# andygrove/datafusion-archive

Hardware: NVIDIA H100
Metric: rows/s filter+agg over 1e8-row Arrow batch (C2: SELECT a FROM t WHERE a>0.5, Float64) (higher is better)
Workload: dtype f64

## Files before the change

datafusion_archive_b200/csrc/api.cu:

```cuda
#include <dlfcn.h>
#include <nccl.h>
#include <sched.h>
#include <sys/syscall.h>
#include <unistd.h>

#include <algorithm>
#include <memory>

#include "common.cuh"

namespace dfgpu {

static thread_local std::string g_last_error;
void set_last_error(const std::string& m) { g_last_error = m; }

const char* dtype_name(int dt) {
  switch (dt) {
    case DFGPU_BOOL: return "Boolean";
    case DFGPU_INT8: return "Int8";
    case DFGPU_INT16: return "Int16";
    case DFGPU_INT32: return "Int32";
    case DFGPU_INT64: return "Int64";
    case DFGPU_UINT8: return "UInt8";
    case DFGPU_UINT16: return "UInt16";
// ... 104 lines not shown
  if (!prof_on) return -1;
  const int s = prof_next;
  prof_next = (prof_next + 1) % kProfRing;
  if (!prof_ev[s][0]) {
    DF_CUDA(cudaEventCreate(&prof_ev[s][0]));
    DF_CUDA(cudaEventCreate(&prof_ev[s][1]));
  }
  if (prof_pending[s]) {
    float ms = 0;
    DF_CUDA(cudaEventSynchronize(prof_ev[s][1]));
    DF_CUDA(cudaEventElapsedTime(&ms, prof_ev[s][0], prof_ev[s][1]));
    prof_ms += ms;
    prof_n++;
    prof_pending[s] = false;
  }
  DF_CUDA(cudaEventRecord(prof_ev[s][0], stream));
  return s;
}
void dfgpu_ctx::prof_end(int s) {
  if (s < 0) return;
  DF_CUDA(cudaEventRecord(prof_ev[s][1], stream));
  prof_pending[s] = true;
}
void dfgpu_ctx::prof_drain() {
  for (int s = 0; s < kProfRing; s++) {
    if (!prof_pending[s]) continue;
    float ms = 0;
    DF_CUDA(cudaEventSynchronize(prof_ev[s][1]));
    DF_CUDA(cudaEventElapsedTime(&ms, prof_ev[s][0], prof_ev[s][1]));
    prof_ms += ms;
    prof_n++;
    prof_pending[s] = false;
  }
}

extern "C" int dfgpu_profile_enable(dfgpu_ctx* ctx, int on) {
  return guarded([&] {
    ctx->use();
    ctx->prof_drain();
    ctx->prof_on = on != 0;
    ctx->prof_ms = 0.0;
    ctx->prof_n = 0;
  });
}
extern "C" int dfgpu_profile_get(dfgpu_ctx* ctx, double* kernel_ms, int64_t* launches) {
  return guarded([&] {
    ctx->use();
    ctx->prof_drain();
    *kernel_ms = ctx->prof_ms;
    *launches = ctx->prof_n;
  });
}

dfgpu_batch::~dfgpu_batch() {
  if (!ctx || !owns) return;
  cudaSetDevice(ctx->device);
  for (auto& c : cols) {
    ctx->free(c.values);
    ctx->free(c.validity);
    ctx->free(c.offsets);
  }
}
void* dfgpu_ctx::host_alloc(size_t bytes) {
  if (bytes == 0) bytes = 8;
  HostBlock* best = nullptr;
  for (auto& b : host_blocks)
    if (!b.used && b.bytes >= bytes && b.bytes <= 2 * bytes + (1 << 20) && (!best || b.bytes < best->bytes)) best = &b;
  if (best) {
    best->used = true;
    return best->p;
  }
  void* p = nullptr;
  DF_CUDA(cudaMallocHost(&p, bytes));
  host_blocks.push_back(HostBlock{p, bytes, true});
  return p;
}
void dfgpu_ctx::host_release(void* p) {
  for (auto& b : host_blocks)
    if (b.p == p) b.used = false;
}

dfgpu_result::~dfgpu_result() {
  if (!ctx) return;
  cudaSetDevice(ctx->device);
  if (on_host) {
    for (auto& c : cols) ctx->host_release(c.values);
    return;
  }
  for (auto& c : cols) {
    ctx->free(c.values);
    ctx->free(c.validity);
    ctx->free(c.offsets);
  }
}

extern "C" int dfgpu_abi_version(void) { return DFGPU_ABI_VERSION; }
extern "C" const char* dfgpu_last_error(void) { return g_last_error.c_str(); }

extern "C" int dfgpu_device_count(int* out) {
  return guarded([&] {
    int n = 0;
    cudaError_t e = cudaGetDeviceCount(&n);
    if (e != cudaSuccess) {
      cudaGetLastError();
      n = 0;
    }
    *out = n;
  });
}

static void bind_to_gpu_numa_node(int device) {
  if (const char* e = getenv("DFGPU_NUMA")) if (atoi(e) == 0) return;
  char bus[64] = {0};
  if (cudaDeviceGetPCIBusId(bus, sizeof(bus), device) != cudaSuccess) { cudaGetLastError(); return; }
  for (char* c = bus; *c; c++) *c = char(tolower((unsigned char)*c));
  int node = -1;
  {
    FILE* f = fopen((std::string("/sys/bus/pci/devices/") + bus + "/numa_node").c_str(), "r");
    if (!f) return;
    if (fscanf(f, "%d", &node) != 1) node = -1;
    fclose(f);
  }
  if (node < 0) {
    if (getenv("DFGPU_TRACE")) fprintf(stderr, "[dfgpu trace] device %d (%s): sysfs reports no NUMA node\n", device, bus);
    return;
  }
  FILE* f = fopen(("/sys/devices/system/node/node" + std::to_string(node) + "/cpulist").c_str(), "r");
  if (!f) return;
  char list[4096] = {0};
  const bool got = fgets(list, sizeof(list), f) != nullptr;
  fclose(f);
  if (!got) return;
  cpu_set_t set;
  CPU_ZERO(&set);
  int ncpu = 0;
  for (char* tok = strtok(list, ",\n"); tok; tok = strtok(nullptr, ",\n")) {
    int a = 0, b = 0;
// ... 7 lines not shown
  if (getenv("DFGPU_TRACE")) fprintf(stderr, "[dfgpu trace] device %d (%s) -> NUMA node %d, %d cpus, sched_setaffinity rc=%d\n", device, bus, node, ncpu, rc_aff);
  unsigned long mask[16] = {0};
  if (node < int(sizeof(mask) * 8)) {
    mask[node / (8 * sizeof(unsigned long))] |= 1ul << (node % (8 * sizeof(unsigned long)));
    syscall(SYS_set_mempolicy, 1 , mask, sizeof(mask) * 8);
  }
}

extern "C" int dfgpu_init(int device, dfgpu_ctx** out) {
  return guarded([&] {
    if (!out) fail(DFGPU_ERR_GENERAL, "dfgpu_init: null out");
    int n = 0;
    cudaError_t e = cudaGetDeviceCount(&n);
    if (e != cudaSuccess || n == 0) {
      cudaGetLastError();
      fail(DFGPU_ERR_CUDA, "no CUDA device available: this engine has no CPU fallback");
    }
    if (device < 0 || device >= n) fail(DFGPU_ERR_CUDA, "device ordinal " + std::to_string(device) + " out of range");
    auto ctx = std::make_unique<dfgpu_ctx>();
    ctx->device = device;
    ctx->use();
    bind_to_gpu_numa_node(device);
    cudaDeviceProp prop;
    DF_CUDA(cudaGetDeviceProperties(&prop, device));
    if (prop.major != 9 || prop.minor != 0)
      fail(DFGPU_ERR_CUDA, std::string("device '") + prop.name + "' is sm_" + std::to_string(prop.major * 10 + prop.minor) +
                               "; this library is built for sm_90a (H100) only");
    ctx->sm_count = prop.multiProcessorCount;
    ctx->device_mem_bytes = prop.totalGlobalMem;
    if (const char* e = getenv("DFGPU_FP_KERNEL")) ctx->force_direct_kernel = std::string(e) == "direct";
    DF_CUDA(cudaStreamCreateWithFlags(&ctx->stream, cudaStreamNonBlocking));
    DF_CUDA(cudaStreamCreateWithFlags(&ctx->stream_in, cudaStreamNonBlocking));
    DF_CUDA(cudaStreamCreateWithFlags(&ctx->stream_out, cudaStreamNonBlocking));
    DF_CUDA(cudaEventCreate(&ctx->ev_start));
    DF_CUDA(cudaEventCreate(&ctx->ev_stop));
    cudaMemPool_t pool;
    DF_CUDA(cudaDeviceGetDefaultMemPool(&pool, device));
    uint64_t thresh = ~0ull;
    DF_CUDA(cudaMemPoolSetAttribute(pool, cudaMemPoolAttrReleaseThreshold, &thresh));
    DF_CUDA(cudaMalloc(&ctx->d_scratch, 64 * 8));
    DF_CUDA(cudaMemset(ctx->d_scratch, 0, 64 * 8));
    DF_CUDA(cudaMallocHost(&ctx->h_scratch, 64 * 8));
    *out = ctx.release();
  });
}

extern "C" int dfgpu_comm_destroy(dfgpu_ctx* ctx);

extern "C" int dfgpu_shutdown(dfgpu_ctx* ctx) {
  return guarded([&] {
    if (!ctx) return;
    ctx->use();
    cudaStreamSynchronize(ctx->stream);
    dfgpu_comm_destroy(ctx);
    ctx->release_cached();
    if (ctx->flush_buf) cudaFree(ctx->flush_buf);
    for (int i = 0; i < 2; i++) {
      if (ctx->stage[i]) cudaFreeHost(ctx->stage[i]);
      if (ctx->stage_ev[i]) cudaEventDestroy(ctx->stage_ev[i]);
    }
    for (int i = 0; i < dfgpu_ctx::kProfRing; i++)
      for (int j = 0; j < 2; j++)
        if (ctx->prof_ev[i][j]) cudaEventDestroy(ctx->prof_ev[i][j]);
    for (auto& b : ctx->host_blocks) cudaFreeHost(b.p);
    cudaStreamDestroy(ctx->stream_in);
    cudaStreamDestroy(ctx->stream_out);
    cudaFree(ctx->d_scratch);
    cudaFreeHost(ctx->h_scratch);
    cudaEventDestroy(ctx->ev_start);
    cudaEventDestroy(ctx->ev_stop);
    cudaStreamDestroy(ctx->stream);
    delete ctx;
  });
}

extern "C" int dfgpu_sync(dfgpu_ctx* ctx) {
  return guarded([&] {
    ctx->use();
    DF_CUDA(cudaStreamSynchronize(ctx->stream));
  });
}

extern "C" int dfgpu_host_alloc(size_t bytes, void** out) {
  return guarded([&] { DF_CUDA(cudaMallocHost(out, bytes ? bytes : 8)); });
}
extern "C" int dfgpu_host_free(void* p) {
  return guarded([&] {
    if (p) DF_CUDA(cudaFreeHost(p));
  });
}

extern "C" int dfgpu_timer_start(dfgpu_ctx* ctx) {
  return guarded([&] {
    ctx->use();
    DF_CUDA(cudaEventRecord(ctx->ev_start, ctx->stream));
  });
}
extern "C" int dfgpu_timer_stop(dfgpu_ctx* ctx, float* ms) {
  return guarded([&] {
    ctx->use();
    DF_CUDA(cudaEventRecord(ctx->ev_stop, ctx->stream));
    DF_CUDA(cudaEventSynchronize(ctx->ev_stop));
    DF_CUDA(cudaEventElapsedTime(ms, ctx->ev_start, ctx->ev_stop));
  });
}

// ... 85 lines not shown
        for (uint8_t byte : tmp) valid += __builtin_popcount(byte);
        d.null_count = c.len - valid;
        if (d.null_count > 0) {
          d.validity = (uint8_t*)ctx->alloc(tmp.size());
          h2d(ctx, d.validity, tmp.data(), tmp.size());
          DF_CUDA(cudaStreamSynchronize(ctx->stream));
        }
      }
      const int w = dtype_width(c.dtype);
      if (w > 0) {
        d.values_bytes = size_t(c.len) * size_t(w);
        d.values = ctx->alloc(d.values_bytes);
        if (c.len > 0) {
          if (!c.values) fail(DFGPU_ERR_GENERAL, "null values buffer");
          h2d(ctx, d.values, static_cast<const uint8_t*>(c.values) + size_t(c.offset) * size_t(w), d.values_bytes);
        }
      } else if (c.dtype == DFGPU_BOOL) {
        std::vector<uint8_t> bits = c.len > 0 ? rebase_bits(static_cast<const uint8_t*>(c.values), c.offset, c.len) : std::vector<uint8_t>();
        d.values_bytes = bits.size();
        d.values = ctx->alloc(d.values_bytes);
        if (!bits.empty()) {
          h2d(ctx, d.values, bits.data(), bits.size());
          DF_CUDA(cudaStreamSynchronize(ctx->stream));
        }
      } else if (c.dtype == DFGPU_UTF8) {
        if (!c.offsets) fail(DFGPU_ERR_GENERAL, "Utf8 column without offsets buffer");
        d.offsets = (int32_t*)ctx->alloc(size_t(c.len + 1) * 4);
        h2d(ctx, d.offsets, c.offsets + c.offset, size_t(c.len + 1) * 4);
        const int32_t lo = c.offsets[c.offset], hi = c.offsets[c.offset + c.len];
        if (hi < lo || hi > c.values_bytes) fail(DFGPU_ERR_GENERAL, "corrupt Utf8 offsets");
        d.values_bytes = size_t(hi - lo);
        d.values = ctx->alloc((d.values_bytes + 15) & ~size_t(15));
        if (hi > lo) h2d(ctx, d.values, static_cast<const uint8_t*>(c.values) + lo, size_t(hi - lo));
        rebase_offsets(ctx, d.offsets, c.len + 1, lo);
      } else {
        fail(DFGPU_ERR_NOT_IMPLEMENTED, std::string("unsupported column type ") + std::to_string(c.dtype));
      }
      b->cols.push_back(d);
    }
    DF_CUDA(cudaStreamSynchronize(ctx->stream));
    *out = b.release();
  });
}

extern "C" int dfgpu_batch_rows(const dfgpu_batch* b, int64_t* nrows) {
  *nrows = b->nrows;
  return 0;
}
extern "C" int dfgpu_batch_free(dfgpu_batch* b) {
  return guarded([&] { delete b; });
}

extern "C" int dfgpu_result_shape(const dfgpu_result* r, int64_t* nrows, int* ncols) {
  *nrows = r->nrows;
  *ncols = int(r->cols.size());
  return 0;
}
extern "C" int dfgpu_result_col_dtype(const dfgpu_result* r, int i, int32_t* dtype) {
  return guarded([&] {
    if (i < 0 || size_t(i) >= r->cols.size()) fail(DFGPU_ERR_INVALID_COLUMN, "result column out of range");
    *dtype = r->cols[size_t(i)].dtype;
  });
}
extern "C" int dfgpu_result_col_bytes(const dfgpu_result* r, int i, int64_t* nbytes) {
  return guarded([&] {
    if (i < 0 || size_t(i) >= r->cols.size()) fail(DFGPU_ERR_INVALID_COLUMN, "result column out of range");
    const DevColumn& c = r->cols[size_t(i)];
    const int w = dtype_width(c.dtype);
    *nbytes = w ? r->nrows * w : int64_t(c.values_bytes);
  });
}
extern "C" int dfgpu_result_col_nulls(const dfgpu_result* r, int i, int64_t* nulls) {
  return guarded([&] {
    if (i < 0 || size_t(i) >= r->cols.size()) fail(DFGPU_ERR_INVALID_COLUMN, "result column out of range");
    *nulls = r->cols[size_t(i)].null_count;
  });
}
extern "C" int dfgpu_result_copy_col(const dfgpu_result* r, int i, void* dst_values, uint8_t* dst_validity, int32_t* dst_offsets) {
  return guarded([&] {
    if (i < 0 || size_t(i) >= r->cols.size()) fail(DFGPU_ERR_INVALID_COLUMN, "result column out of range");
    dfgpu_ctx* ctx = r->ctx;
    ctx->use();
    const DevColumn& c = r->cols[size_t(i)];
    const int w = dtype_width(c.dtype);
    const size_t nb = w ? size_t(r->nrows) * size_t(w) : c.values_bytes;
    if (r->on_host) {
      if (nb && dst_values) memcpy(dst_values, c.values, nb);
      if (dst_validity) memset(dst_validity, 0xff, size_t(r->nrows + 7) / 8);
      return;
    }
    if (nb && dst_values) DF_CUDA(cudaMemcpyAsync(dst_values, c.values, nb, cudaMemcpyDeviceToHost, ctx->stream));
    if (dst_validity) {
      const size_t vb = size_t(r->nrows + 7) / 8;
      if (c.validity) DF_CUDA(cudaMemcpyAsync(dst_validity, c.validity, vb, cudaMemcpyDeviceToHost, ctx->stream));
      else memset(dst_validity, 0xff, vb);
    }
    if (dst_offsets && c.offsets)
      DF_CUDA(cudaMemcpyAsync(dst_offsets, c.offsets, size_t(r->nrows + 1) * 4, cudaMemcpyDeviceToHost, ctx->stream));
    DF_CUDA(cudaStreamSynchronize(ctx->stream));
  });
}
extern "C" int dfgpu_result_col_device_ptr(const dfgpu_result* r, int i, const void** dptr) {
  return guarded([&] {
    if (i < 0 || size_t(i) >= r->cols.size()) fail(DFGPU_ERR_INVALID_COLUMN, "result column out of range");
    if (r->on_host) fail(DFGPU_ERR_GENERAL, "result lives in host memory: use dfgpu_result_col_host_ptr");
    *dptr = r->cols[size_t(i)].values;
  });
}
extern "C" int dfgpu_result_on_host(const dfgpu_result* r, int* on_host) {
  return guarded([&] {
    if (!r || !on_host) fail(DFGPU_ERR_GENERAL, "dfgpu_result_on_host: null argument");
    *on_host = r->on_host ? 1 : 0;
  });
}
extern "C" int dfgpu_result_col_host_ptr(const dfgpu_result* r, int i, const void** hptr) {
  return guarded([&] {
    if (i < 0 || size_t(i) >= r->cols.size()) fail(DFGPU_ERR_INVALID_COLUMN, "result column out of range");
    if (!r->on_host) fail(DFGPU_ERR_GENERAL, "result lives in device memory: use dfgpu_result_copy_col");
    *hptr = r->cols[size_t(i)].values;
  });
}
extern "C" int dfgpu_result_free(dfgpu_result* r) {
  return guarded([&] { delete r; });
}

namespace {

struct NcclApi {
  void* h = nullptr;
  ncclResult_t (*GetUniqueId)(ncclUniqueId*) = nullptr;
  ncclResult_t (*CommInitRank)(ncclComm_t*, int, ncclUniqueId, int) = nullptr;
  ncclResult_t (*CommDestroy)(ncclComm_t) = nullptr;
  ncclResult_t (*AllGather)(const void*, void*, size_t, ncclDataType_t, ncclComm_t, cudaStream_t) = nullptr;
  ncclResult_t (*AllReduce)(const void*, void*, size_t, ncclDataType_t, ncclRedOp_t, ncclComm_t, cudaStream_t) = nullptr;
  ncclResult_t (*Send)(const void*, size_t, ncclDataType_t, int, ncclComm_t, cudaStream_t) = nullptr;
  ncclResult_t (*Recv)(void*, size_t, ncclDataType_t, int, ncclComm_t, cudaStream_t) = nullptr;
  ncclResult_t (*Broadcast)(const void*, void*, size_t, ncclDataType_t, int, ncclComm_t, cudaStream_t) = nullptr;
  ncclResult_t (*GroupStart)() = nullptr;
  ncclResult_t (*GroupEnd)() = nullptr;
  const char* (*GetErrorString)(ncclResult_t) = nullptr;
};

NcclApi& nccl() {
  static NcclApi api;
  if (api.h) return api;
  void* h = dlopen("libnccl.so.2", RTLD_NOW | RTLD_NOLOAD);
  if (!h) h = dlopen("libnccl.so.2", RTLD_NOW);
  if (!h) h = dlopen("libnccl.so", RTLD_NOW);
  if (!h) fail(DFGPU_ERR_CUDA, std::string("cannot load libnccl: ") + dlerror());
#define LOAD(N)                                                     \
  *(void**)(&api.N) = dlsym(h, "nccl" #N);                          \
  if (!api.N) fail(DFGPU_ERR_CUDA, "libnccl is missing symbol nccl" #N);
  LOAD(GetUniqueId) LOAD(CommInitRank) LOAD(CommDestroy) LOAD(AllGather) LOAD(AllReduce) LOAD(GroupStart) LOAD(GroupEnd)
  LOAD(Send) LOAD(Recv) LOAD(Broadcast)
  LOAD(GetErrorString)
#undef LOAD
  api.h = h;
  return api;
}

#define DF_NCCL(expr)                                                                                        \
  do {                                                                                                       \
    ncclResult_t _r = (expr);                                                                                \
    if (_r != ncclSuccess) fail(DFGPU_ERR_CUDA, std::string("NCCL error: ") + nccl().GetErrorString(_r) + " (" #expr ")"); \
  } while (0)

}

extern "C" int dfgpu_comm_unique_id(uint8_t out_id[128]) {
  return guarded([&] {
    static_assert(sizeof(ncclUniqueId) == 128, "ncclUniqueId size");
// ... 115 lines not shown
```

datafusion_archive_b200/csrc/common.cuh:

```cuda
#pragma once
#include <cuda_runtime.h>

#include <cstdint>
#include <cstdio>
#include <cstring>
#include <string>
#include <map>
#include <unordered_map>
#include <vector>

#include "../../include/dfgpu.h"

namespace dfgpu {

struct Error {
  int code;
  std::string msg;
};
[[noreturn]] inline void fail(int code, const std::string& m) { throw Error{code, m}; }

void set_last_error(const std::string& m);

#define DF_CUDA(expr)                                                                              \
  do {                                                                                             \
// ... 13 lines not shown
    set_last_error(e.msg);
    return e.code;
  } catch (const std::exception& e) {
    set_last_error(std::string("internal: ") + e.what());
    return DFGPU_ERR_INTERNAL;
  }
}

const char* dtype_name(int dt);
int dtype_width(int dt);
inline bool is_signed_int(int dt) { return dt >= DFGPU_INT8 && dt <= DFGPU_INT64; }
inline bool is_unsigned_int(int dt) { return dt >= DFGPU_UINT8 && dt <= DFGPU_UINT64; }
inline bool is_int(int dt) { return dt >= DFGPU_INT8 && dt <= DFGPU_UINT64; }
inline bool is_float(int dt) { return dt == DFGPU_FLOAT32 || dt == DFGPU_FLOAT64; }
inline bool is_numeric(int dt) { return dt >= DFGPU_INT8 && dt <= DFGPU_FLOAT64; }
inline bool is_numeric8(int dt) { return dt == DFGPU_FLOAT64 || dt == DFGPU_INT64 || dt == DFGPU_UINT64; }
inline bool is_numeric4or8(int dt) { return is_numeric8(dt) || dt == DFGPU_FLOAT32 || dt == DFGPU_INT32 || dt == DFGPU_UINT32; }

}

struct dfgpu_ctx {
  int device = 0;
  int sm_count = 132;
  size_t device_mem_bytes = 0;
  cudaStream_t stream = nullptr;
  cudaEvent_t ev_start = nullptr, ev_stop = nullptr;
  int64_t launches = 0;
  bool force_direct_kernel = false;
  void* flush_buf = nullptr;
  size_t flush_bytes = 0;
  unsigned long long* d_scratch = nullptr;
  unsigned long long* h_scratch = nullptr;
  void* stage[2] = {nullptr, nullptr};
  cudaEvent_t stage_ev[2] = {nullptr, nullptr};
  size_t stage_bytes = 0;
  static constexpr int kProfRing = 32;
  bool prof_on = false;
  cudaEvent_t prof_ev[kProfRing][2] = {};
  bool prof_pending[kProfRing] = {};
  int prof_next = 0;
  double prof_ms = 0.0;
  int64_t prof_n = 0;
  int prof_begin();
  void prof_end(int slot);
  void prof_drain();
  cudaStream_t stream_in = nullptr, stream_out = nullptr;
  struct HostBlock { void* p; size_t bytes; bool used; };
  std::vector<HostBlock> host_blocks;
  void* host_alloc(size_t bytes);
  void host_release(void* p);
  int rank = 0, world = 1;
  void* nccl_comm = nullptr;

  std::vector<const void*> configured_kernels;
  bool first_use(const void* kernel) {
    for (const void* k : configured_kernels)
      if (k == kernel) return false;
    configured_kernels.push_back(kernel);
    return true;
  }

  static constexpr size_t kBigBlock = 256u << 10;
  std::map<size_t, std::vector<void*>> big_free;
  std::unordered_map<void*, size_t> big_live;
  size_t big_cached_bytes = 0;
  void release_cached();
  void* alloc(size_t bytes);
  void free(void* p);
  void use();
};

struct DevColumn {
  int dtype = 0;
  void* values = nullptr;
  size_t values_bytes = 0;
  uint8_t* validity = nullptr;
  int32_t* offsets = nullptr;
  int64_t null_count = 0;
};

namespace dfgpu {
void comm_allgather_u64(dfgpu_ctx* ctx, const unsigned long long* send, unsigned long long* recv, size_t count);
void comm_exchange_v(dfgpu_ctx* ctx, const unsigned long long* send, const size_t* send_off, const size_t* send_cnt,
                     unsigned long long* recv, const size_t* recv_off, const size_t* recv_cnt);
void comm_allgather_v(dfgpu_ctx* ctx, const unsigned long long* send, unsigned long long* recv, const size_t* off, const size_t* cnt);
void comm_allgather_bytes_v(dfgpu_ctx* ctx, const void* send, void* recv, const size_t* off, const size_t* cnt);
void comm_allreduce_aggs(dfgpu_ctx* ctx, int naggs, const int* funcs, const int* mtypes, unsigned long long* d_vals, unsigned long long* d_nonnull,
                         unsigned long long* d_rows);
struct Utf8Source {
  const int* off;
  const unsigned char* bytes;
};
constexpr int UTF8_SRC_SHIFT = 40;

struct Trace {
  bool on;
  dfgpu_ctx* ctx;
  double t0;
  explicit Trace(dfgpu_ctx* c);
  void mark(const char* what);
};
void trace_launch(const char* kernel);
}

struct dfgpu_batch {
  dfgpu_ctx* ctx = nullptr;
  int64_t nrows = 0;
  std::vector<DevColumn> cols;
  bool owns = true;
  ~dfgpu_batch();
};

struct dfgpu_result {
  dfgpu_ctx* ctx = nullptr;
  int64_t nrows = 0;
  std::vector<DevColumn> cols;
  bool on_host = false;
  ~dfgpu_result();
};
```

datafusion_archive_b200/csrc/expr_vm.cuh:

```cuda
#pragma once
#include "common.cuh"

namespace dfgpu {

enum MType : uint8_t { MT_NONE = 0, MT_F64 = 1, MT_F32 = 2, MT_I = 3, MT_U = 4, MT_BOOL = 5 };
enum VOp : uint8_t {
  V_PUSH_COL = 0, V_PUSH_IMM, V_PUSH_ROWID , V_CAST,
  V_ADD, V_SUB, V_MUL, V_DIV,
  V_EQ, V_NE, V_LT, V_LE, V_GT, V_GE,
  V_AND, V_OR,
  V_RSUB, V_RDIV,
  V_FN, V_FN2, V_RFN2
};
constexpr int kFnDepth = 9;
inline std::string depth_arg(int depth) { return depth == kFnDepth ? "kFnDepth" : std::to_string(depth); }
enum RhsMode : uint8_t { RHS_STACK = 0, RHS_IMM = 1, RHS_COL = 2 };

struct __align__(16) DevInsn {
  uint8_t op;
  uint8_t mode;
  uint8_t mtype;
  uint8_t dtype;
  int16_t slot;
  int16_t aux;
  unsigned long long imm;
};

constexpr int kMaxInsn = 96;
constexpr int kMaxProgs = 24;
constexpr int kMaxCols = 12;

struct ColRef {
  const void* ptr;
  const unsigned char* validity;
  int dtype;
  int _pad;
};

struct ProgramSet {
  DevInsn insn[kMaxInsn];
  ColRef cols[kMaxCols];
  uint8_t start[kMaxProgs + 1];
  uint8_t out_dtype[kMaxProgs];
  int nprog;
  int ncols;
  int max_depth;
  int f64_only;
  int has_nulls;
  uint8_t nullable[kMaxProgs];
};
inline bool has_fn(const ProgramSet& ps) {
  for (int pc = 0; pc < ps.start[ps.nprog]; pc++)
    if (ps.insn[pc].op >= V_FN) return true;
  return false;
}

struct Leaf {
  int kind;
  int op;
  int a, b;
  int dtype;
  uint8_t mtype;
  uint8_t conn;
  unsigned long long imm;
};
struct LeafChain {
  int nterms;
  Leaf term[4];
};
static_assert(sizeof(Leaf) == 32 && sizeof(LeafChain) == 136, "FPParams and AggParams carry chains and leaves: keep them compact");

struct CompiledProgram {
  std::vector<DevInsn> code;
  bool nullable = false;
  int out_dtype = 0;
  int max_depth = 0;
  Leaf leaf{};
  LeafChain chain{};
};

struct Utf8Pred {
  int op;
  int a, b;
  std::string lit;
  int synth;
};

constexpr int kMaxUtf8Steps = 16;
struct Utf8Step {
  int op;
  long long start;
  long long count;
};
struct Utf8ViewSpec {
  int nsteps;
  int case_map;
  int result;
  Utf8Step step[kMaxUtf8Steps];
};
struct Utf8View {
  int src;
  Utf8ViewSpec spec;
  int synth;
  bool projection;
  DevColumn out;
};
// ... 499 lines not shown
```

datafusion_archive_b200/csrc/filter_project.cu:

```cuda
#include <memory>

#include "filter_project.cuh"

namespace dfgpu {

template <int DEPTH, bool NULLS>
__global__ void __launch_bounds__(FP_THREADS) k_filter_project(const __grid_constant__ FPParams p) {
  __shared__ int s_tile;
  __shared__ unsigned s_wcount[FP_ITEMS * FP_WARPS];
  __shared__ unsigned s_woff[FP_ITEMS * FP_WARPS];
  __shared__ unsigned long long s_prefix;
  static_assert(FP_ITEMS * FP_WARPS == 64, "scan below assumes 64 (item,warp) counters = 2 per lane");

  const int tid = threadIdx.x, lane = tid & 31, warp = tid >> 5;
  const unsigned lt_mask = (1u << lane) - 1u;

  for (;;) {
    if (tid == 0) s_tile = (int)atomicAdd(p.ticket, 1u);
    __syncthreads();
    const int tile = s_tile;
    if (tile >= p.ntiles) break;
    const long long base = (long long)tile * FP_TILE;

    unsigned flags = 0;
// ... 261 lines not shown
    for (int i = 0; i < nproj; i++) {
      DevColumn c;
      if (out_kind[size_t(i)] >= 0) {
        c.dtype = pb.out_dtype(out_kind[size_t(i)] + has_pred);
        if (c.dtype == DFGPU_BOOL) {
          DevColumn b;
          b.dtype = DFGPU_UINT8;
          b.values_bytes = size_t(n > 0 ? n : 1);
          b.values = ctx->alloc(b.values_bytes);
          bool_of_out[size_t(i)] = int(bool_bytes.cols.size());
          bool_bytes.cols.push_back(b);
          kern_out[size_t(out_kind[size_t(i)])] = b.values;
          c.values_bytes = size_t((n + 31) / 32) * 4 + 4;
          c.values = ctx->alloc(c.values_bytes);
        } else {
          c.values_bytes = size_t(n > 0 ? n : 1) * size_t(dtype_width(c.dtype));
          c.values = ctx->alloc(c.values_bytes);
          kern_out[size_t(out_kind[size_t(i)])] = c.values;
        }
      } else {
        c.dtype = DFGPU_UTF8;
      }
      res->cols.push_back(c);
    }
    if (rowid_slot >= 0) {
      DevColumn c;
      c.dtype = DFGPU_UINT64;
      c.values_bytes = size_t(n > 0 ? n : 1) * 8;
      c.values = ctx->alloc(c.values_bytes);
      scratch.cols.push_back(c);
      kern_out[size_t(rowid_slot)] = c.values;
    }
    if (n == 0) {
      for (auto& c : res->cols)
        if (c.dtype == DFGPU_BOOL) c.values_bytes = 0;
      for (auto& c : res->cols)
        if (c.dtype == DFGPU_UTF8) {
          c.offsets = (int32_t*)ctx->alloc(4);
          DF_CUDA(cudaMemsetAsync(c.offsets, 0, 4, ctx->stream));
          c.values = ctx->alloc(1);
        }
      DF_CUDA(cudaStreamSynchronize(ctx->stream));
      res->nrows = 0;
      *out = res.release();
      return;
    }
    p.nrows = n;
    p.has_pred = has_pred;
    p.nproj = nkern;
    for (int i = 0; i < nkern; i++) p.out[i] = kern_out[size_t(i)];
    const size_t max_tiles = size_t((n + 1023) / 1024) + 1;
    unsigned long long* status = (unsigned long long*)ctx->alloc((max_tiles + 8) * 8);
    DF_CUDA(cudaMemsetAsync(status, 0, (max_tiles + 8) * 8, ctx->stream));
    ctx->h_scratch[0] = 0;
    ctx->h_scratch[2] = 0;
    p.tile_status = status + 8;
    p.ticket = (unsigned*)(status + 0);
    p.out_count = ctx->h_scratch + 0;
    p.err_flag = (unsigned*)(ctx->h_scratch + 2);
    memset(p.out_valid, 0, sizeof(p.out_valid));
    p.null_counts = ctx->d_scratch + 32;
    std::vector<int> valid_of_out(size_t(nproj), -1);
    if (p.ps.has_nulls && !has_pred) {
      DF_CUDA(cudaMemsetAsync(ctx->d_scratch + 32, 0, kMaxProgs * 8, ctx->stream));
      for (int i = 0; i < nproj; i++) {
        const int k = out_kind[size_t(i)];
        if (k >= 0 && p.ps.nullable[k]) {
          const size_t vbytes = size_t((n + 31) / 32) * 4;
          res->cols[size_t(i)].validity = (uint8_t*)ctx->alloc(vbytes);
          DF_CUDA(cudaMemsetAsync(res->cols[size_t(i)].validity, 0, vbytes, ctx->stream));
          p.out_valid[k] = (unsigned*)res->cols[size_t(i)].validity;
          valid_of_out[size_t(i)] = k;
        }
      }
    }
    p.pred_fast = has_pred ? pb.prog(0).chain : LeafChain{};
    for (int i = 0; i < nkern; i++) p.proj_fast[i] = pb.prog(i + has_pred).leaf;
    const bool fn = has_fn(p.ps);
    if (p.ps.has_nulls) {
      p.ntiles = int((n + FP_TILE - 1) / FP_TILE);
      if (fn) launch_fp<kFnDepth, true>(ctx, p);
      else launch_fp<8, true>(ctx, p);
    } else if (ctx->force_direct_kernel || !launch_fp_tma(ctx, p)) {
      p.ntiles = int((n + FP_TILE - 1) / FP_TILE);
      const int d = p.ps.max_depth;
      if (fn) launch_fp<kFnDepth>(ctx, p);
      else if (d <= 1) launch_fp<1>(ctx, p);
      else if (d <= 2) launch_fp<2>(ctx, p);
      else if (d <= 4) launch_fp<4>(ctx, p);
      else launch_fp<8>(ctx, p);
    }
    if (p.ps.has_nulls && !has_pred)
      DF_CUDA(cudaMemcpyAsync(ctx->h_scratch + 32, ctx->d_scratch + 32, kMaxProgs * 8, cudaMemcpyDeviceToHost, ctx->stream));
    DF_CUDA(cudaStreamSynchronize(ctx->stream));
    ctx->free(status);
    for (int i = 0; i < nproj; i++) {
      DevColumn& c = res->cols[size_t(i)];
      if (valid_of_out[size_t(i)] >= 0) {
        c.null_count = (int64_t)ctx->h_scratch[32 + valid_of_out[size_t(i)]];
        if (c.null_count == 0) {
          ctx->free(c.validity);
          c.validity = nullptr;
        }
      }
    }
    if ((unsigned)ctx->h_scratch[2] != 0) fail(DFGPU_ERR_ARROW, "DivideByZero");
    res->nrows = has_pred ? (int64_t)ctx->h_scratch[0] : n;
    for (int i = 0; i < nproj; i++)
      if (bool_of_out[size_t(i)] >= 0) {
        DevColumn& c = res->cols[size_t(i)];
        const long long words = (res->nrows + 31) / 32;
        if (words > 0) {
          k_pack_bits<<<grid_for_rows(ctx, words * 32), 256, 0, ctx->stream>>>(
              (const unsigned char*)bool_bytes.cols[size_t(bool_of_out[size_t(i)])].values, res->nrows, (unsigned*)c.values);
          DF_CUDA(cudaGetLastError());
          ctx->launches++;
        }
        c.values_bytes = size_t(res->nrows + 7) / 8;
        any_utf8 = true;
      }
    for (int i = 0; i < nproj; i++)
      if (out_view[size_t(i)] >= 0)
        pb.eval_utf8_view_rows(ctx, out_view[size_t(i)], has_pred ? (const unsigned long long*)scratch.cols[0].values : nullptr, res->nrows,
                               &res->cols[size_t(i)]);
      else if (out_kind[size_t(i)] < 0)
        gather_utf8(ctx, batch->cols[size_t(-1 - out_kind[size_t(i)])], (const unsigned long long*)scratch.cols[0].values, res->nrows,
                    &res->cols[size_t(i)]);
    if (!has_pred)
      for (int i = 0; i < nproj; i++)
        if (out_kind[size_t(i)] < 0) {
          const int src = out_view[size_t(i)] >= 0 ? pb.utf8_views()[size_t(out_view[size_t(i)])].src : -1 - out_kind[size_t(i)];
          const DevColumn& srcc = batch->cols[size_t(src)];
          if (srcc.null_count > 0) {
            const size_t vb = size_t(n + 7) / 8;
            res->cols[size_t(i)].validity = (uint8_t*)ctx->alloc(vb);
            DF_CUDA(cudaMemcpyAsync(res->cols[size_t(i)].validity, srcc.validity, vb, cudaMemcpyDeviceToDevice, ctx->stream));
            res->cols[size_t(i)].null_count = srcc.null_count;
          }
        }
    if (any_utf8) DF_CUDA(cudaStreamSynchronize(ctx->stream));
    *out = res.release();
  });
}
// ... 98 lines not shown
    for (long long c = 0; c < nchunks; c++) {
      auto ch = std::make_unique<Chunk>();
      ch->batch.ctx = ctx;
      const long long r0 = c * (long long)chunk_rows, rows = std::min<long long>((long long)chunk_rows, n - r0);
      ch->batch.nrows = rows > 0 ? rows : 0;
      for (int u : used) {
        DevColumn d;
        d.dtype = cols[u].dtype;
        d.values_bytes = size_t(ch->batch.nrows) * size_t(dtype_width(d.dtype));
        d.values = ctx->alloc(d.values_bytes);
        ch->batch.cols.push_back(d);
      }
      DF_CUDA(cudaEventCreateWithFlags(&ch->ev, cudaEventDisableTiming));
      chunks.push_back(std::move(ch));
    }
    DF_CUDA(cudaEventRecord(ev_alloc, ctx->stream));
    DF_CUDA(cudaStreamWaitEvent(ctx->stream_in, ev_alloc, 0));
    cudaEventDestroy(ev_alloc);
    for (long long c = 0; c < nchunks; c++) {
      Chunk& ch = *chunks[size_t(c)];
      const long long r0 = c * chunk_rows;
      for (size_t k = 0; k < used.size(); k++) {
        const dfgpu_col& hc = cols[used[k]];
        const int w = dtype_width(hc.dtype);
        if (ch.batch.nrows > 0)
          DF_CUDA(cudaMemcpyAsync(ch.batch.cols[k].values, static_cast<const uint8_t*>(hc.values) + size_t(hc.offset + r0) * size_t(w),
                                  size_t(ch.batch.nrows) * size_t(w), cudaMemcpyHostToDevice, ctx->stream_in));
      }
      DF_CUDA(cudaEventRecord(ch.ev, ctx->stream_in));
    }
    auto res = std::make_unique<dfgpu_result>();
    res->ctx = ctx;
    res->on_host = true;
    long long off = 0;
    for (long long c = 0; c < nchunks; c++) {
      Chunk& ch = *chunks[size_t(c)];
      DF_CUDA(cudaStreamWaitEvent(ctx->stream, ch.ev, 0));
      int rc = dfgpu_filter_project(ctx, &ch.batch, pred2.data(), int(pred2.size()), proj2p.data(), proj2l.data(), nproj, &ch.res);
      if (rc != 0) fail(rc, dfgpu_last_error());
      if (c == 0) {
        for (int q = 0; q < nproj; q++) {
          DevColumn hcol;
          hcol.dtype = ch.res->cols[size_t(q)].dtype;
          if (!is_numeric(hcol.dtype)) {
            resident = true;
            break;
          }
          hcol.values_bytes = size_t(n > 0 ? n : 1) * size_t(dtype_width(hcol.dtype));
          hcol.values = ctx->host_alloc(hcol.values_bytes);
          res->cols.push_back(hcol);
        }
      }
      if (resident) break;
      for (int q = 0; q < nproj; q++) {
        const int w = dtype_width(res->cols[size_t(q)].dtype);
        if (ch.res->nrows > 0)
          DF_CUDA(cudaMemcpyAsync(static_cast<uint8_t*>(res->cols[size_t(q)].values) + size_t(off) * size_t(w), ch.res->cols[size_t(q)].values,
                                  size_t(ch.res->nrows) * size_t(w), cudaMemcpyDeviceToHost, ctx->stream_out));
      }
      off += ch.res->nrows;
    }
    DF_CUDA(cudaStreamSynchronize(ctx->stream_out));
    if (resident) {
      res.reset();
      run_resident();
      return;
    }
    res->nrows = off;
    *out = res.release();
  });
}
```

datafusion_archive_b200/engine.py:

```python
import ctypes as C
import os
import subprocess

import numpy as np

from . import _abi as A

_LIB = None


class DfGpuError(Exception):
    def __init__(self, code, msg):
        super().__init__("dfgpu error %d: %s" % (code, msg))
        self.code, self.msg = code, msg


def lib_path():
    return os.environ.get("DFGPU_LIB") or os.path.join(os.path.dirname(os.path.abspath(__file__)), "libdfgpu.so")


def build(force=False):
    here = os.path.dirname(os.path.abspath(__file__))
    csrc = os.path.join(here, "csrc")
    so = lib_path()
# ... 35 lines not shown
    L.dfgpu_filter_project_host.argtypes = [vp, C.POINTER(A.Col), C.c_int, PI, C.c_int, C.POINTER(PI), C.POINTER(C.c_int), C.c_int, C.c_int64, C.POINTER(vp)]
    L.dfgpu_result_col_host_ptr.argtypes = [vp, C.c_int, C.POINTER(vp)]
    L.dfgpu_result_on_host.argtypes = [vp, C.POINTER(C.c_int)]
    L.dfgpu_aggregate_create.argtypes = [vp, C.POINTER(PI), C.POINTER(C.c_int), C.c_int, C.POINTER(A.Agg), C.c_int, C.c_int64, C.POINTER(vp)]
    L.dfgpu_aggregate_set_predicate.argtypes = [vp, PI, C.c_int]
    L.dfgpu_aggregate_update.argtypes = [vp, vp]
    L.dfgpu_aggregate_update_host.argtypes = [vp, C.POINTER(A.Col), C.c_int, C.c_int64]
    L.dfgpu_aggregate_finish.argtypes = [vp, C.POINTER(vp)]
    L.dfgpu_aggregate_free.argtypes = [vp]
    L.dfgpu_result_shape.argtypes = [vp, C.POINTER(C.c_int64), C.POINTER(C.c_int)]
    L.dfgpu_result_col_dtype.argtypes = [vp, C.c_int, C.POINTER(C.c_int32)]
    L.dfgpu_result_col_bytes.argtypes = [vp, C.c_int, C.POINTER(C.c_int64)]
    L.dfgpu_result_col_nulls.argtypes = [vp, C.c_int, C.POINTER(C.c_int64)]
    L.dfgpu_result_copy_col.argtypes = [vp, C.c_int, vp, vp, vp]
    L.dfgpu_result_col_device_ptr.argtypes = [vp, C.c_int, C.POINTER(vp)]
    L.dfgpu_result_free.argtypes = [vp]
    L.dfgpu_comm_unique_id.argtypes = [C.c_char_p]
    L.dfgpu_comm_init.argtypes = [vp, C.c_int, C.c_int, C.c_char_p]
    L.dfgpu_comm_destroy.argtypes = [vp]
    PC = C.POINTER(C.c_int)
    L.dfgpu_join_build.argtypes = [vp, vp, C.POINTER(PI), PC, C.c_int, PC, C.c_int, C.POINTER(vp)]
    L.dfgpu_join_probe.argtypes = [vp, vp, C.POINTER(PI), PC, C.c_int, PC, C.c_int, PC, C.c_int, C.POINTER(vp)]
    L.dfgpu_join_semi.argtypes = [vp, vp, C.POINTER(PI), PC, C.c_int, C.c_int, PC, C.c_int, C.POINTER(vp)]
    L.dfgpu_join_free.argtypes = [vp]
    if L.dfgpu_abi_version() != A.ABI_VERSION:
        raise RuntimeError("libdfgpu.so ABI version mismatch")
    _LIB = L
    return L


def check(rc):
    if rc != 0:
        raise DfGpuError(rc, lib().dfgpu_last_error().decode())


class PinnedBuffer:

    def __init__(self, shape, dtype):
        self.dtype = np.dtype(dtype)
        n = int(np.prod(shape))
        self.ptr = C.c_void_p()
        check(lib().dfgpu_host_alloc(max(8, n * self.dtype.itemsize), C.byref(self.ptr)))
        buf = (C.c_uint8 * (n * self.dtype.itemsize)).from_address(self.ptr.value)
        self.array = np.frombuffer(buf, dtype=self.dtype, count=n).reshape(shape)

    def free(self):
        if self.ptr:
            self.array = None
            lib().dfgpu_host_free(self.ptr)
            self.ptr = None


class Result:
    def __init__(self, ctx, handle):
        self.ctx, self.h = ctx, handle
        nrows, ncols = C.c_int64(), C.c_int()
        lib().dfgpu_result_shape(self.h, C.byref(nrows), C.byref(ncols))
        self.nrows, self.ncols = nrows.value, ncols.value

    def dtype(self, i):
        dt = C.c_int32()
        check(lib().dfgpu_result_col_dtype(self.h, i, C.byref(dt)))
        return dt.value

    @property
    def on_host(self):
        f = C.c_int()
        check(lib().dfgpu_result_on_host(self.h, C.byref(f)))
        return bool(f.value)

    def host_view(self, i):
        p = C.c_void_p()
        check(lib().dfgpu_result_col_host_ptr(self.h, i, C.byref(p)))
        dt = np.dtype(A.NP_OF[self.dtype(i)])
        buf = (C.c_uint8 * (self.nrows * dt.itemsize)).from_address(p.value) if self.nrows else (C.c_uint8 * 0)()
        return np.frombuffer(buf, dtype=dt, count=self.nrows)

    def copy_into(self, i, dst):
        check(lib().dfgpu_result_copy_col(self.h, i, dst.ctypes.data, None, None))

    def columns(self):
        from_fetch = _fetch_result(lib(), self.h)
        return from_fetch

    def free(self):
        if self.h:
            if self.ctx.h:
                check(lib().dfgpu_result_free(self.h))
            self.h = None

    def __del__(self):
        try:
            self.free()
        except Exception:
            pass


def _fetch_result(L, handle):
    nrows, ncols = C.c_int64(), C.c_int()
    L.dfgpu_result_shape(handle, C.byref(nrows), C.byref(ncols))
    n = nrows.value
    cols = []
    for i in range(ncols.value):
        dt, nulls = C.c_int32(), C.c_int64()
        check(L.dfgpu_result_col_dtype(handle, i, C.byref(dt)))
        check(L.dfgpu_result_col_nulls(handle, i, C.byref(nulls)))
        validity = np.zeros((n + 7) // 8, dtype=np.uint8) if nulls.value else None
        vptr = validity.ctypes.data if validity is not None else None
        if dt.value == A.UTF8:
            nb = C.c_int64()
            check(L.dfgpu_result_col_bytes(handle, i, C.byref(nb)))
            data = np.zeros(max(1, nb.value), dtype=np.uint8)
            offs = np.zeros(n + 1, dtype=np.int32)
            check(L.dfgpu_result_copy_col(handle, i, data.ctypes.data, vptr, offs.ctypes.data))
            raw = data.tobytes()
            vals = [raw[offs[k]:offs[k + 1]].decode() for k in range(n)]
        elif dt.value == A.BOOL:
            packed = np.zeros(max(1, (n + 7) // 8), dtype=np.uint8)
            check(L.dfgpu_result_copy_col(handle, i, packed.ctypes.data, vptr, None))
            vals = np.unpackbits(packed, bitorder="little")[:n].astype(bool)
        else:
            vals = np.zeros(max(1, n), dtype=A.NP_OF[dt.value])
            check(L.dfgpu_result_copy_col(handle, i, vals.ctypes.data, vptr, None))
            vals = vals[:n]
        if validity is not None:
            cols.append((vals, np.unpackbits(validity, bitorder="little")[:n].astype(bool)))
        else:
            cols.append(vals)
    return cols


def check_program(schema_dtypes, expr):
    prog = expr.program(list(schema_dtypes))
    arr = (A.Insn * max(1, len(prog)))(*prog)
    dts = (C.c_int32 * max(1, len(schema_dtypes)))(*schema_dtypes)
    out = C.c_int32()
    L = lib()
    L.dfgpu_check_program.argtypes = [C.POINTER(C.c_int32), C.c_int, C.POINTER(A.Insn), C.c_int, C.POINTER(C.c_int32)]
    check(L.dfgpu_check_program(dts, len(schema_dtypes), arr, len(prog), C.byref(out)))
    return out.value


def utf8_like_host(s, pattern):
    s = s.encode("utf-8") if isinstance(s, str) else bytes(s)
    pattern = pattern.encode("utf-8") if isinstance(pattern, str) else bytes(pattern)
    m, cls = C.c_int32(), C.c_int32()
    L = lib()
    L.dfgpu_utf8_like_host.argtypes = [C.c_char_p, C.c_int64, C.c_char_p, C.c_int64, C.POINTER(C.c_int32), C.POINTER(C.c_int32)]
    check(L.dfgpu_utf8_like_host(s, len(s), pattern, len(pattern), C.byref(m), C.byref(cls)))
    return bool(m.value), cls.value


def utf8_fn_host(s, expr):
# ... 1 lines not shown
    prog = expr.program([A.UTF8])
    arr = (A.Insn * len(prog))(*prog)
    out = C.create_string_buffer(max(1, len(s)))
    out_len, out_int, out_dtype = C.c_int64(), C.c_int64(), C.c_int32()
    L = lib()
    L.dfgpu_utf8_fn_host.argtypes = [C.c_char_p, C.c_int64, C.POINTER(A.Insn), C.c_int, C.c_char_p, C.POINTER(C.c_int64),
                                     C.POINTER(C.c_int64), C.POINTER(C.c_int32)]
    check(L.dfgpu_utf8_fn_host(s, len(s), arr, len(prog), out, C.byref(out_len), C.byref(out_int), C.byref(out_dtype)))
    return out.raw[:out_len.value] if out_dtype.value == A.UTF8 else out_int.value


class Batch:
    def __init__(self, ctx, handle, schema):
        self.ctx, self.h, self.schema = ctx, handle, schema
        n = C.c_int64()
        lib().dfgpu_batch_rows(self.h, C.byref(n))
        self.nrows = n.value

    def free(self):
        if self.h:
            if self.ctx.h:
                check(lib().dfgpu_batch_free(self.h))
            self.h = None

    def __del__(self):
        try:
            self.free()
        except Exception:
            pass


class GpuContext:

    def __init__(self, device=0):
        self.h = C.c_void_p()
        check(lib().dfgpu_init(device, C.byref(self.h)))
        self.device = device

    def upload(self, arrays):
        keep = []
        cols = A.make_cols(arrays, keep)
        out = C.c_void_p()
        check(lib().dfgpu_batch_upload(self.h, cols, len(arrays), C.byref(out)))
        return Batch(self, out, [cols[i].dtype for i in range(len(arrays))])

    def filter_project(self, batch, pred=None, proj=()):
        schema = batch.schema
        pprog = pred.program(schema) if pred is not None else []
        parr = (A.Insn * max(1, len(pprog)))(*pprog)
        keep = []
        ptrs, lens, n = A.make_programs([e.program(schema) for e in proj], keep)
        out = C.c_void_p()
        check(lib().dfgpu_filter_project(self.h, batch.h, parr, len(pprog), ptrs, lens, n, C.byref(out)))
        return Result(self, out)

    def filter_project_host(self, arrays, pred=None, proj=(), chunk_rows=0):
        keep = []
        cols = A.make_cols(arrays, keep)
        schema = [cols[i].dtype for i in range(len(arrays))]
        pprog = pred.program(schema) if pred is not None else []
        parr = (A.Insn * max(1, len(pprog)))(*pprog)
        ptrs, lens, n = A.make_programs([e.program(schema) for e in proj], keep)
        out = C.c_void_p()
        check(lib().dfgpu_filter_project_host(self.h, cols, len(arrays), parr, len(pprog), ptrs, lens, n, chunk_rows, C.byref(out)))
        return Result(self, out)

    def aggregate(self, batches, keys=(), aggs=(), expected_groups=0, pred=None):
        if isinstance(batches, Batch):
            batches = [batches]
        schema = batches[0].schema
        keep = []
        kptrs, klens, nk = A.make_programs([k.program(schema) for k in keys], keep)
        aggarr = A.make_aggs([a.lower(schema) for a in aggs], keep)
        st = C.c_void_p()
        check(lib().dfgpu_aggregate_create(self.h, kptrs, klens, nk, aggarr, len(aggs), expected_groups, C.byref(st)))
        try:
            if pred is not None:
                pprog = pred.program(schema)
                parr = (A.Insn * max(1, len(pprog)))(*pprog)
                check(lib().dfgpu_aggregate_set_predicate(st, parr, len(pprog)))
            for b in batches:
                check(lib().dfgpu_aggregate_update(st, b.h))
            out = C.c_void_p()
            check(lib().dfgpu_aggregate_finish(st, C.byref(out)))
            return Result(self, out)
        finally:
            lib().dfgpu_aggregate_free(st)

    def aggregate_host(self, arrays, keys=(), aggs=(), expected_groups=0, pred=None, chunk_rows=0):
        keep = []
        cols = A.make_cols(arrays, keep)
        schema = [cols[i].dtype for i in range(len(arrays))]
        kptrs, klens, nk = A.make_programs([k.program(schema) for k in keys], keep)
        aggarr = A.make_aggs([a.lower(schema) for a in aggs], keep)
        st = C.c_void_p()
        check(lib().dfgpu_aggregate_create(self.h, kptrs, klens, nk, aggarr, len(aggs), expected_groups, C.byref(st)))
        try:
            if pred is not None:
                pprog = pred.program(schema)
                parr = (A.Insn * max(1, len(pprog)))(*pprog)
                check(lib().dfgpu_aggregate_set_predicate(st, parr, len(pprog)))
            check(lib().dfgpu_aggregate_update_host(st, cols, len(arrays), chunk_rows))
            out = C.c_void_p()
            check(lib().dfgpu_aggregate_finish(st, C.byref(out)))
            return Result(self, out)
        finally:
            lib().dfgpu_aggregate_free(st)
# ... 95 lines not shown
```

Baseline: 212.8 billion.

## Make filter_project return stream-ordered with lazy row-count resolution

```diff
diff --git a/datafusion_archive_b200/csrc/api.cu b/datafusion_archive_b200/csrc/api.cu
--- a/datafusion_archive_b200/csrc/api.cu
+++ b/datafusion_archive_b200/csrc/api.cu
@@ -180,6 +180,70 @@
   });
 }
 
+int dfgpu_ctx::fp_acquire(dfgpu_result* owner) {
+  if (fp_free.empty()) {
+    for (size_t i = 0; i < fp_retired.size();) {
+      const cudaError_t e = cudaEventQuery(fp_slots[size_t(fp_retired[i])].done);
+      if (e == cudaErrorNotReady) {
+        cudaGetLastError();
+        i++;
+        continue;
+      }
+      DF_CUDA(e);
+      fp_free.push_back(fp_retired[i]);
+      fp_retired[i] = fp_retired.back();
+      fp_retired.pop_back();
+    }
+  }
+  if (fp_free.empty()) {
+    unsigned long long* words = nullptr;
+    DF_CUDA(cudaMallocHost(&words, size_t(kFpSlab) * 2 * 8));
+    fp_slabs.push_back(words);
+    for (int i = 0; i < kFpSlab; i++) {
+      FpSlot s;
+      s.words = words + 2 * i;
+      DF_CUDA(cudaEventCreateWithFlags(&s.done, cudaEventDisableTiming));
+      fp_free.push_back(int(fp_slots.size()));
+      fp_slots.push_back(s);
+    }
+  }
+  const int s = fp_free.back();
+  fp_free.pop_back();
+  FpSlot& slot = fp_slots[size_t(s)];
+  slot.words[0] = 0;
+  slot.words[1] = 0;
+  slot.owner = owner;
+  return s;
+}
+
+void dfgpu_ctx::fp_retire(int s) {
+  fp_slots[size_t(s)].owner = nullptr;
+  fp_retired.push_back(s);
+}
+
+namespace dfgpu {
+
+static void settle(const dfgpu_result* r) {
+  dfgpu_ctx* ctx = r->ctx;
+  dfgpu_ctx::FpSlot& s = ctx->fp_slots[size_t(r->pending)];
+  DF_CUDA(cudaEventSynchronize(s.done));
+  r->nrows = (int64_t)s.words[0];
+  r->div_by_zero = s.words[1] != 0;
+  s.owner = nullptr;
+  ctx->fp_free.push_back(r->pending);
+  r->pending = -1;
+}
+
+void resolve(const dfgpu_result* r) {
+  if (r->pending >= 0) {
+    r->ctx->use();
+    settle(r);
+  }
+  if (r->div_by_zero) fail(DFGPU_ERR_ARROW, "DivideByZero");
+}
+
+}
+
 dfgpu_batch::~dfgpu_batch() {
   if (!ctx || !owns) return;
   cudaSetDevice(ctx->device);
@@ -211,6 +275,7 @@
 dfgpu_result::~dfgpu_result() {
   if (!ctx) return;
   cudaSetDevice(ctx->device);
+  if (pending >= 0) ctx->fp_retire(pending);
   if (on_host) {
     for (auto& c : cols) ctx->host_release(c.values);
     return;
@@ -324,6 +389,10 @@
     if (!ctx) return;
     ctx->use();
     cudaStreamSynchronize(ctx->stream);
+    for (auto& s : ctx->fp_slots)
+      if (s.owner) settle(s.owner);
+    for (auto& s : ctx->fp_slots) cudaEventDestroy(s.done);
+    for (void* w : ctx->fp_slabs) cudaFreeHost(w);
     dfgpu_comm_destroy(ctx);
     ctx->release_cached();
     if (ctx->flush_buf) cudaFree(ctx->flush_buf);
@@ -515,9 +584,11 @@
 }
 
 extern "C" int dfgpu_result_shape(const dfgpu_result* r, int64_t* nrows, int* ncols) {
-  *nrows = r->nrows;
-  *ncols = int(r->cols.size());
-  return 0;
+  return guarded([&] {
+    resolve(r);
+    *nrows = r->nrows;
+    *ncols = int(r->cols.size());
+  });
 }
 extern "C" int dfgpu_result_col_dtype(const dfgpu_result* r, int i, int32_t* dtype) {
   return guarded([&] {
@@ -528,6 +599,7 @@
 extern "C" int dfgpu_result_col_bytes(const dfgpu_result* r, int i, int64_t* nbytes) {
   return guarded([&] {
     if (i < 0 || size_t(i) >= r->cols.size()) fail(DFGPU_ERR_INVALID_COLUMN, "result column out of range");
+    resolve(r);
     const DevColumn& c = r->cols[size_t(i)];
     const int w = dtype_width(c.dtype);
     *nbytes = w ? r->nrows * w : int64_t(c.values_bytes);
@@ -536,12 +608,14 @@
 extern "C" int dfgpu_result_col_nulls(const dfgpu_result* r, int i, int64_t* nulls) {
   return guarded([&] {
     if (i < 0 || size_t(i) >= r->cols.size()) fail(DFGPU_ERR_INVALID_COLUMN, "result column out of range");
+    resolve(r);
     *nulls = r->cols[size_t(i)].null_count;
   });
 }
 extern "C" int dfgpu_result_copy_col(const dfgpu_result* r, int i, void* dst_values, uint8_t* dst_validity, int32_t* dst_offsets) {
   return guarded([&] {
     if (i < 0 || size_t(i) >= r->cols.size()) fail(DFGPU_ERR_INVALID_COLUMN, "result column out of range");
+    resolve(r);
     dfgpu_ctx* ctx = r->ctx;
     ctx->use();
     const DevColumn& c = r->cols[size_t(i)];
@@ -567,6 +641,7 @@
   return guarded([&] {
     if (i < 0 || size_t(i) >= r->cols.size()) fail(DFGPU_ERR_INVALID_COLUMN, "result column out of range");
     if (r->on_host) fail(DFGPU_ERR_GENERAL, "result lives in host memory: use dfgpu_result_col_host_ptr");
+    resolve(r);
     *dptr = r->cols[size_t(i)].values;
   });
 }
@@ -580,6 +655,7 @@
   return guarded([&] {
     if (i < 0 || size_t(i) >= r->cols.size()) fail(DFGPU_ERR_INVALID_COLUMN, "result column out of range");
     if (!r->on_host) fail(DFGPU_ERR_GENERAL, "result lives in device memory: use dfgpu_result_copy_col");
+    resolve(r);
     *hptr = r->cols[size_t(i)].values;
   });
 }
diff --git a/datafusion_archive_b200/csrc/common.cuh b/datafusion_archive_b200/csrc/common.cuh
--- a/datafusion_archive_b200/csrc/common.cuh
+++ b/datafusion_archive_b200/csrc/common.cuh
@@ -89,6 +89,19 @@
   int rank = 0, world = 1;
   void* nccl_comm = nullptr;
 
+  struct FpSlot {
+    unsigned long long* words = nullptr;
+    cudaEvent_t done = nullptr;
+    dfgpu_result* owner = nullptr;
+  };
+  static constexpr int kFpSlab = 64;
+  std::vector<FpSlot> fp_slots;
+  std::vector<void*> fp_slabs;
+  std::vector<int> fp_free;
+  std::vector<int> fp_retired;
+  int fp_acquire(dfgpu_result* owner);
+  void fp_retire(int slot);
+
   std::vector<const void*> configured_kernels;
   bool first_use(const void* kernel) {
     for (const void* k : configured_kernels)
@@ -150,8 +163,14 @@
 
 struct dfgpu_result {
   dfgpu_ctx* ctx = nullptr;
-  int64_t nrows = 0;
+  mutable int64_t nrows = 0;
+  mutable int pending = -1;
+  mutable bool div_by_zero = false;
   std::vector<DevColumn> cols;
   bool on_host = false;
   ~dfgpu_result();
 };
+
+namespace dfgpu {
+void resolve(const dfgpu_result* r);
+}
diff --git a/datafusion_archive_b200/csrc/expr_vm.cuh b/datafusion_archive_b200/csrc/expr_vm.cuh
--- a/datafusion_archive_b200/csrc/expr_vm.cuh
+++ b/datafusion_archive_b200/csrc/expr_vm.cuh
@@ -52,6 +52,11 @@
 inline bool has_fn(const ProgramSet& ps) {
   for (int pc = 0; pc < ps.start[ps.nprog]; pc++)
     if (ps.insn[pc].op >= V_FN) return true;
+  return false;
+}
+inline bool has_div(const ProgramSet& ps) {
+  for (int pc = 0; pc < ps.start[ps.nprog]; pc++)
+    if (ps.insn[pc].op == V_DIV || ps.insn[pc].op == V_RDIV) return true;
   return false;
 }
 
diff --git a/datafusion_archive_b200/csrc/filter_project.cu b/datafusion_archive_b200/csrc/filter_project.cu
--- a/datafusion_archive_b200/csrc/filter_project.cu
+++ b/datafusion_archive_b200/csrc/filter_project.cu
@@ -337,12 +337,21 @@
     const size_t max_tiles = size_t((n + 1023) / 1024) + 1;
     unsigned long long* status = (unsigned long long*)ctx->alloc((max_tiles + 8) * 8);
     DF_CUDA(cudaMemsetAsync(status, 0, (max_tiles + 8) * 8, ctx->stream));
-    ctx->h_scratch[0] = 0;
-    ctx->h_scratch[2] = 0;
     p.tile_status = status + 8;
     p.ticket = (unsigned*)(status + 0);
-    p.out_count = ctx->h_scratch + 0;
-    p.err_flag = (unsigned*)(ctx->h_scratch + 2);
+    bool any_bool = false;
+    for (int i = 0; i < nproj; i++) any_bool = any_bool || bool_of_out[size_t(i)] >= 0;
+    const bool stream_ordered = has_pred && !p.ps.has_nulls && !any_utf8 && !any_bool && !has_div(p.ps);
+    if (stream_ordered) {
+      res->pending = ctx->fp_acquire(res.get());
+      p.out_count = ctx->fp_slots[size_t(res->pending)].words;
+      p.err_flag = (unsigned*)(p.out_count + 1);
+    } else {
+      ctx->h_scratch[0] = 0;
+      ctx->h_scratch[2] = 0;
+      p.out_count = ctx->h_scratch + 0;
+      p.err_flag = (unsigned*)(ctx->h_scratch + 2);
+    }
     memset(p.out_valid, 0, sizeof(p.out_valid));
     p.null_counts = ctx->d_scratch + 32;
     std::vector<int> valid_of_out(size_t(nproj), -1);
@@ -374,6 +383,13 @@
       else if (d <= 2) launch_fp<2>(ctx, p);
       else if (d <= 4) launch_fp<4>(ctx, p);
       else launch_fp<8>(ctx, p);
+    }
+    if (stream_ordered) {
+      DF_CUDA(cudaEventRecord(ctx->fp_slots[size_t(res->pending)].done, ctx->stream));
+      ctx->free(status);
+      if (getenv("DFGPU_TRACE")) fprintf(stderr, "[dfgpu trace] filter_project returns stream-ordered\n");
+      *out = res.release();
+      return;
     }
     if (p.ps.has_nulls && !has_pred)
       DF_CUDA(cudaMemcpyAsync(ctx->h_scratch + 32, ctx->d_scratch + 32, kMaxProgs * 8, cudaMemcpyDeviceToHost, ctx->stream));
@@ -578,6 +594,7 @@
         }
       }
       if (resident) break;
+      resolve(ch.res);
       for (int q = 0; q < nproj; q++) {
         const int w = dtype_width(res->cols[size_t(q)].dtype);
         if (ch.res->nrows > 0)
diff --git a/datafusion_archive_b200/engine.py b/datafusion_archive_b200/engine.py
--- a/datafusion_archive_b200/engine.py
+++ b/datafusion_archive_b200/engine.py
@@ -111,11 +111,29 @@
 
 
 class Result:
-    def __init__(self, ctx, handle):
+
+    def __init__(self, ctx, handle, shape_on_first_use=False):
         self.ctx, self.h = ctx, handle
-        nrows, ncols = C.c_int64(), C.c_int()
-        lib().dfgpu_result_shape(self.h, C.byref(nrows), C.byref(ncols))
-        self.nrows, self.ncols = nrows.value, ncols.value
+        self._shape = None
+        if not shape_on_first_use:
+            self._read_shape()
+
+    def _read_shape(self):
+        if self._shape is None:
+            if not self.h:
+                raise RuntimeError("the result was freed before its shape was read")
+            nrows, ncols = C.c_int64(), C.c_int()
+            check(lib().dfgpu_result_shape(self.h, C.byref(nrows), C.byref(ncols)))
+            self._shape = (nrows.value, ncols.value)
+        return self._shape
+
+    @property
+    def nrows(self):
+        return self._read_shape()[0]
+
+    @property
+    def ncols(self):
+        return self._read_shape()[1]
 
     def dtype(self, i):
         dt = C.c_int32()
@@ -157,7 +175,7 @@
 
 def _fetch_result(L, handle):
     nrows, ncols = C.c_int64(), C.c_int()
-    L.dfgpu_result_shape(handle, C.byref(nrows), C.byref(ncols))
+    check(L.dfgpu_result_shape(handle, C.byref(nrows), C.byref(ncols)))
     n = nrows.value
     cols = []
     for i in range(ncols.value):
@@ -265,7 +283,7 @@
         ptrs, lens, n = A.make_programs([e.program(schema) for e in proj], keep)
         out = C.c_void_p()
         check(lib().dfgpu_filter_project(self.h, batch.h, parr, len(pprog), ptrs, lens, n, C.byref(out)))
-        return Result(self, out)
+        return Result(self, out, shape_on_first_use=True)
 
     def filter_project_host(self, arrays, pred=None, proj=(), chunk_rows=0):
         keep = []
diff --git a/profiles/microbench_fp_steps.py b/profiles/microbench_fp_steps.py
--- /dev/null
+++ b/profiles/microbench_fp_steps.py
@@ -0,0 +1,94 @@
+#!/usr/bin/env python
+import argparse
+import json
+import os
+import subprocess
+import sys
+
+import numpy as np
+
+ROOT = os.path.dirname(os.path.dirname(os.path.abspath(__file__)))
+sys.path.insert(0, ROOT)
+
+
+def one_run(args):
+    from datafusion_archive_b200 import engine, workloads
+    ctx = engine.GpuContext(0)
+    out = {"lib": engine.lib_path(), "rows": args.rows, "steps": args.steps}
+    a2, pred2, proj2 = workloads.c2(args.rows, seed=42)
+    a3, pred3, proj3 = workloads.c3(args.rows, seed=142)
+    shapes = {"c2": (a2, pred2, proj2, int(np.count_nonzero(a2[0] > 0.5))),
+              "c3": (a3[:2], pred3, proj3, int(np.count_nonzero(a3[1] < a3[0])))}
+    for name, (arrays, pred, proj, nsel) in shapes.items():
+        batch = ctx.upload(arrays)
+        held = [None]
+
+        def step():
+            r = ctx.filter_project(batch, pred, proj)
+            if held[0] is not None:
+                held[0].free()
+            held[0] = r
+        for _ in range(args.warmup):
+            step()
+        ctx.sync()
+        ctx.profile_enable(True)
+        ctx.timer_start()
+        for _ in range(args.steps):
+            step()
+        ms = ctx.timer_stop()
+        kms, kn = ctx.profile_get()
+        ctx.profile_enable(False)
+        assert held[0].nrows == nsel, "%s: %d rows, expected %d" % (name, held[0].nrows, nsel)
+        held[0].free()
+        batch.free()
+        out[name] = {"step_ms": ms / args.steps, "kernel_ms": kms / kn, "gap_ms": ms / args.steps - kms / kn, "launches": kn}
+    ctx.close()
+    print(json.dumps(out))
+
+
+def gpu_info():
+    try:
+        return subprocess.run(["nvidia-smi", "-i", "0", "--query-gpu=name,power.limit,clocks.max.sm", "--format=csv,noheader"],
+                              capture_output=True, text=True, timeout=30).stdout.strip()
+    except Exception as e:
+        return "nvidia-smi failed: %r" % e
+
+
+def ab(args):
+    libs = args.ab
+    runs = {lib: [] for lib in libs}
+    base = [sys.executable, os.path.abspath(__file__), "--rows", str(args.rows), "--steps", str(args.steps), "--warmup", str(args.warmup)]
+    for rnd in range(args.rounds):
+        for lib in libs:
+            env = dict(os.environ, DFGPU_LIB=os.path.abspath(lib))
+            line = subprocess.run(base, env=env, capture_output=True, text=True, check=True).stdout.strip().splitlines()[-1]
+            runs[lib].append(json.loads(line))
+            print("round %d %s: %s" % (rnd, lib, line), file=sys.stderr, flush=True)
+    summary = {"gpu": gpu_info(), "rows": args.rows, "steps": args.steps, "warmup": args.warmup, "rounds": args.rounds, "libs": {}}
+    for lib in libs:
+        s = {}
+        for shape in ("c2", "c3"):
+            s[shape] = {}
+            for key in ("step_ms", "kernel_ms", "gap_ms"):
+                v = [r[shape][key] for r in runs[lib]]
+                s[shape][key] = {"median": float(np.median(v)), "min": float(min(v)), "max": float(max(v))}
+        summary["libs"][lib] = s
+    print(json.dumps(summary, indent=1))
+
+
+def main():
+    ap = argparse.ArgumentParser()
+    ap.add_argument("--rows", type=int, default=100_000_000)
+    ap.add_argument("--steps", type=int, default=100)
+    ap.add_argument("--warmup", type=int, default=5)
+    ap.add_argument("--ab", nargs=2, metavar="LIB", default=None)
+    ap.add_argument("--rounds", type=int, default=5)
+    args = ap.parse_args()
+    if args.ab:
+        ab(args)
+    else:
+        one_run(args)
+
+
+if __name__ == "__main__":
+    main()
```

Result: faster. 231.5 billion, median of 6 (+8.8%).
